# wcy199705/DfFintheWild

Hardware: AMD Instinct MI355X
Metric: focal-stacks/sec (10x3x256x256) (higher is better)
Workload: dtype bf16x3 (split-bf16 MFMA operands hi+lo, fp32 accumulate, fp32-accurate); 1 GPU; DFF_net forward, 10-slice 3x256x256 focal stacks, batch 32 per GPU (BASELINE.json config 3), dense focus_dists, synthetic weights seed 0; batch_per_gpu=32, global_batch=32, slices=10, height=256, width=256, parallelism=single GPU, precision=bf16x3, input=float32 (B,3,N,H,W), the reference's tensor contract

## Files before the change

dffinthewild_amd/csrc/dffw_conv_tile.h:

```cpp
#pragma once
#include "dffw_internal.h"

namespace dffw {

enum Geo {
    G3S1 = 0,
    G3S2 = 1,
    G3T = 2,
    G2S1 = 3,
    G2D = 4,
    G2S2 = 5,
    G2P = 6,
    GEO_COUNT = 6
};

struct GeoInfo {
    int minz, maxz, miny, maxy, minx, maxx;
    int s;
    int os;
    int npass;
};

inline GeoInfo geo_info(int geo) {
    switch (geo) {
        case G3S1: return GeoInfo{-1, 1, -1, 1, -1, 1, 1, 1, 1};
        case G3S2: return GeoInfo{-1, 1, -1, 1, -1, 1, 2, 1, 1};
        case G3T: return GeoInfo{-1, 1, 0, 1, 0, 1, 1, 2, 4};
        case G2D: return GeoInfo{0, 0, -8, 8, -6, 10, 1, 1, 1};
        case G2S2: return GeoInfo{0, 0, -1, 1, -1, 1, 2, 1, 1};
        case G2P: return GeoInfo{0, 0, -8, 8, -6, 10, 1, 1, 1};
        default: return GeoInfo{0, 0, -1, 1, -1, 1, 1, 1, 1};
    }
}

struct TileCfg {
    int id;
    int geo, nt, cg;
    int tz, ty, tx;
    int fz, fy, fx, fxl;
    int pipe;
    int nw;
    int kt;
    bool lean;
};

struct TileArgs {
    int npass, nstage;
    int KC[4];
    const int *tab[4];
    const uint16_t *wpk[4];
    int ooy[4], oox[4];
    int tiles_z, tiles_y, tiles_x;
    int total_tiles;
    int nt_total;
    int nsplit;
    int grid;
    int pass_split;
    int ksplit;
    float *partial;
    int64_t partial_stride;
    int warm;
};

enum class TileVariant { PLAIN, LEAN, SPLITK, RAW, SUMS };
constexpr int TILE_VARIANTS = 5;

const TileCfg *tile_cfg_find(int geo, int nt, int cg, bool wide = false);
const TileCfg *tile_cfg_find_shape(int geo, int nt, int cg, int tz, int ty, int tx);
const TileCfg *tile_cfg_find_like(const TileCfg *base, int nt);
const TileCfg *tile_cfg_find_team(const TileCfg *base, int nstage, int nt);
bool tile_cfg_has_splitk(const TileCfg *c);
bool tile_cfg_has_sums(const TileCfg *c);
int tile_cfg_count();
const TileCfg *tile_cfg_at(int i);
hipError_t launch_conv_tile(int prec, const TileCfg *cfg, const ConvArgs &a, const TileArgs &t, hipStream_t s);
void conv_tile_kernel_name(int prec, const TileCfg *cfg, const ConvArgs &a, const TileArgs &t, char *buf, int n);

}
```

dffinthewild_amd/csrc/dffw_conv_tile.hip:

```cpp
#include <cstdio>
#include <cstdlib>
#include <initializer_list>

#include "dffw_conv_geom.h"

#ifndef DFFW_TILE_PREC
#error "compile with -DDFFW_TILE_PREC=0|1|2 (arithmetic of this object, see the Makefile)"
#endif

namespace dffw {

template <int PREC, int GEO, int NT, int TZ, int TY, int TX, int CG, int PIPE, int NWAVES = 4, bool SPLITK = false, bool LEAN = false, int KT = 1>
__global__ __launch_bounds__(NWAVES * KT * 64) void conv_tile(const ConvArgs a, const TileArgs t) {
    using T = TileT<GEO, TZ, TY, TX, CG>;
    using G = GeoT<GEO>;
    constexpr int PARTS = Fmt<PREC>::PARTS;
    constexpr bool F16 = (PREC == P_FP16);
    constexpr int MTW = T::MT / NWAVES;
    constexpr bool STEM = (GEO == G2D || GEO == G2P);
    constexpr bool STEMP = (GEO == G2P);
    constexpr bool SUMS = (GEO == G2S1) && SPLITK;
    constexpr int CG8 = CG / 8;

    constexpr int PIXB = CG * 2;
    constexpr int PLANEB = (T::FPIX * PIXB + 1023) / 1024 * 1024;
    constexpr int LDSB = PARTS * PLANEB;
    static_assert(PLANEB < 65536, "lo-plane offset must fit the ds_read immediate");
    static_assert(KT == 1 || (!SPLITK && GEO != G2D && GEO != G2P), "teams: conv geometries (the transposed conv only with its passes split over grid.z), no split-K / raw variants");
    static_assert(KT * LDSB <= 160 * 1024, "the teams' LDS images must fit one CU");
    __shared__ __attribute__((aligned(1024))) unsigned char smem_all[KT * LDSB];

    const int team = KT > 1 ? (int)threadIdx.x / (NWAVES * 64) : 0;
    unsigned char *const smem = smem_all + team * LDSB;
    const int tid = KT > 1 ? (int)threadIdx.x % (NWAVES * 64) : (int)threadIdx.x;
    const int lane = tid & 63;
    const int wave = tid >> 6;
    const int g = lane >> 4, r = lane & 15;
    const int ntb = blockIdx.y * NT;
    const int NTT = t.nt_total;

    int tile;
    {
        const int bid = blockIdx.x;
        const int xcd = bid & 7, idx = bid >> 3;
        const int q = t.total_tiles >> 3, rem = t.total_tiles & 7;
        const int xs = xcd < rem ? xcd * (q + 1) : rem * (q + 1) + (xcd - rem) * q;
        const int xe = xs + q + (xcd < rem ? 1 : 0);
        tile = xs + idx;
        if (tile >= xe) return;
    }

    struct Coord {
        int b, gz0, gy0, gx0;
    };
    auto decode = [&](int tile) {
        Coord c;
        const int txi = tile % t.tiles_x;
        int tt = tile / t.tiles_x;
        const int tyi = tt % t.tiles_y;
        tt /= t.tiles_y;
        const int tzi = tt % t.tiles_z;
        c.b = tt / t.tiles_z;
        c.gz0 = tzi * TZ;
        c.gy0 = tyi * TY;
        c.gx0 = txi * TX;
        return c;
    };

    int pofs[MTW], voff[MTW], tcrd[MTW];
    const int lanepart = (PARTS == 2) ? (g & 1) * a.Cout + (g >> 1) * 8 : g * 4;
#pragma unroll
    for (int j = 0; j < MTW; ++j) {
        const int p = (wave * MTW + j) * 16 + r;
        if constexpr (STEMP) {
            constexpr int HP = TX / 2;
            const int k = p % HP, ty = (p / HP) % TY, tz = p / (HP * TY);
            const int tx = (k & 1) + 4 * (k >> 1) + 2 * (g >> 1);
            pofs[j] = ((tz * T::FY + ty) * T::FXL + k) * PIXB;
            voff[j] = ((tz * a.Ho + ty) * a.Wo + tx) * (PARTS * 8) + ((PARTS == 2) ? (g & 1) * 8 : (g & 1) * 4);
            tcrd[j] = tx | (ty << 8) | (tz << 16);
        } else {
            const int tx = p % TX, ty = (p / TX) % TY, tz = p / (TX * TY);
            pofs[j] = ((tz * T::FY + ty * G::S) * T::FXL + tx) * PIXB;
// ... 142 lines not shown
                uint32_t hh[4], ll[4];
                Fmt<PREC>::split2(px(0, iy, q - 2), px(1, iy, q - 2), hh[0], ll[0]);
                Fmt<PREC>::split2(px(2, iy, q - 2), 0.f, hh[1], ll[1]);
                Fmt<PREC>::split2(px(0, iy, q), px(1, iy, q), hh[2], ll[2]);
                Fmt<PREC>::split2(px(2, iy, q), 0.f, hh[3], ll[3]);
                h = __builtin_bit_cast(short8, (u32x4v){hh[0], hh[1], hh[2], hh[3]});
                l = __builtin_bit_cast(short8, (u32x4v){ll[0], ll[1], ll[2], ll[3]});
            }
            *reinterpret_cast<short8 *>(smem + p * PIXB) = h;
            if constexpr (PARTS == 2) *reinterpret_cast<short8 *>(smem + PLANEB + p * PIXB) = l;
        }
    };
    bool from_stack = false;
    if constexpr (STEM) from_stack = STEMP || a.fs32 != nullptr;
    if (from_stack) {
        if constexpr (STEM) fill_from_stack(cur);
    } else if (!(a.dbg & 1)) {
        issue_fill(cur, st_lo);
    }
    if (t.warm) {
        uint32_t sink = 0;
        const int wstride = NTT * PARTS * 64;
        for (int pass = pass_lo; pass < pass_hi; ++pass) {
            const int KCp = t.KC[pass];
            const int nlines = (st_hi - st_lo) * KCp * NT * PARTS * 8;
            const unsigned char *wb = reinterpret_cast<const unsigned char *>(t.wpk[pass]);
            if (tid * 128 < KCp * 16) {
                const unsigned char *p = reinterpret_cast<const unsigned char *>(t.tab[pass]) + tid * 128;
                asm volatile("global_load_dword %0, %1, off" : "+v"(sink) : "v"(p));
            }
            for (int i = tid; i < nlines; i += NWAVES * 64) {
                const int l8 = i & 7, f = (i >> 3) % (NT * PARTS), c = (i >> 3) / (NT * PARTS);
                const int kc = c % KCp, st = st_lo + c / KCp;
                const unsigned char *p = wb + ((((int64_t)st * KCp + kc) * wstride + ntb * PARTS * 64 + f * 64) * 16 + l8 * 128);
                asm volatile("global_load_dword %0, %1, off" : "+v"(sink) : "v"(p));
            }
        }
        asm volatile("s_waitcnt vmcnt(0)" : "+v"(sink)::"memory");
    }
    stamp(1);

    {
        f32x4 acc[NT][MTW];
#pragma unroll 1
        for (int pass = pass_lo; pass < pass_hi; ++pass) {
#pragma unroll
            for (int nt = 0; nt < NT; ++nt)
#pragma unroll
                for (int j = 0; j < MTW; ++j) acc[nt][j] = (BIAS_IN_ACC && !splitk && team == 0) ? bias4[nt] : f32x4{0.f, 0.f, 0.f, 0.f};

            const int KC = t.KC[pass];
            const int *tab = t.tab[pass] + g;

            for (int sti = st_lo; sti < st_hi; ++sti) {
                const bool backwards = (GEO == G3T) && ((pass - pass_lo) & 1);
                const int st = backwards ? st_hi - 1 - (sti - st_lo) : sti;
                const bool resident = (GEO == G3T) && pass > pass_lo && sti == st_lo && st_hi - st_lo > 1;
                const bool prefilled = (pass == pass_lo && sti == st_lo);
                const int wstride = NTT * PARTS * 64;
                const short8 *wp = reinterpret_cast<const short8 *>(t.wpk[pass]) + (int64_t)st * KC * wstride + ntb * PARTS * 64 + lane;
                short8 wfirst[NT][PARTS];
#pragma unroll
                for (int nt = 0; nt < NT; ++nt)
#pragma unroll
                    for (int pt = 0; pt < PARTS; ++pt) wfirst[nt][pt] = wp[(nt * PARTS + pt) * 64];
                const int tfirst = tab[0];
                constexpr int WD = KT > 1 ? 4 : 1;
                short8 wr[WD][NT][PARTS];
                int tr[WD];
                if constexpr (KT > 1) {
#pragma unroll
                    for (int q = 0; q < WD; ++q) {
                        const int kq = q < KC ? q : KC - 1;
#pragma unroll
                        for (int nt = 0; nt < NT; ++nt)
#pragma unroll
                            for (int pt = 0; pt < PARTS; ++pt) wr[q][nt][pt] = wp[(int64_t)kq * wstride + (nt * PARTS + pt) * 64];
                        tr[q] = tab[kq * 4];
                    }
                }
                if ((pass == pass_lo || st_hi - st_lo > 1) && !resident && !(a.dbg & 1)) {
                    if (!prefilled) {
                        __syncthreads();
                        issue_fill(cur, st);
                    }
                    asm volatile("s_waitcnt vmcnt(0)" ::: "memory");
                    __syncthreads();
                    if (prefilled) stamp(2);
                }

                if constexpr (PIPE == 0) {
                    short8 wf[NT][PARTS], wn[NT][PARTS];
                    int toff = tfirst, tn = 0;
    #pragma unroll
                    for (int nt = 0; nt < NT; ++nt)
    #pragma unroll
                        for (int pt = 0; pt < PARTS; ++pt) wf[nt][pt] = wfirst[nt][pt];
                    for (int kc = 0; kc < ((a.dbg & 2) ? 1 : KC); ++kc) {
                        if (kc + 1 < KC) {
    #pragma unroll
                            for (int nt = 0; nt < NT; ++nt)
    #pragma unroll
                                for (int pt = 0; pt < PARTS; ++pt) wn[nt][pt] = wp[(int64_t)(kc + 1) * wstride + (nt * PARTS + pt) * 64];
                            tn = tab[(kc + 1) * 4];
                        }
    #pragma unroll
// ... 433 lines not shown
    X(9, G3T, 1, 5, 4, 16, 16, 0, 4, 1)    \
    X(10, G3T, 2, 5, 4, 16, 16, 1, 4, 1)   \
    X(11, G3T, 4, 5, 4, 16, 16, 1, 4, 1)   \
    X(12, G2S1, 1, 5, 4, 16, 8, 0, 4, 1)   \
    X(13, G2S1, 1, 5, 4, 16, 16, 0, 4, 1)  \
    X(14, G2S1, 2, 5, 8, 16, 16, 1, 4, 1)  \
    X(15, G2D, 1, 1, 16, 32, 8, 0, 4, 1)   \
    X(16, G3S1, 2, 4, 4, 8, 16, 1, 4, 1)   \
    X(17, G3S2, 2, 4, 4, 8, 8, 1, 4, 1)    \
    X(18, G2S1, 2, 5, 4, 16, 8, 1, 4, 1)   \
    X(19, G2S1, 4, 5, 4, 16, 16, 1, 4, 1)  \
    X(20, G2S1, 4, 5, 4, 16, 8, 1, 4, 1)   \
    X(21, G2S2, 1, 5, 4, 16, 8, 0, 4, 1)   \
    X(22, G2S2, 2, 5, 4, 16, 8, 0, 4, 1)   \
    X(23, G3T, 1, 5, 4, 16, 32, 0, 4, 1)   \
    X(24, G3T, 2, 5, 4, 16, 32, 1, 4, 1)   \
    X(25, G3T, 4, 5, 4, 16, 32, 1, 4, 1)   \
    X(34, G2S1, 2, 5, 4, 16, 32, 1, 4, 1)  \
    X(37, G3S2, 4, 4, 4, 8, 16, 1, 4, 1)   \
    X(38, G3S2, 2, 4, 4, 8, 16, 1, 4, 1)   \
    X(39, G3S2, 1, 4, 4, 8, 16, 1, 4, 1)   \
    X(32, G2P, 1, 1, 16, 32, 8, 0, 4, 1)   \
    X(40, G3S1, 1, 5, 8, 8, 16, 1, 4, 1)   \
    X(41, G3S1, 2, 5, 8, 8, 16, 1, 4, 1)   \
    X(42, G3S1, 4, 5, 8, 8, 16, 1, 4, 1)   \
    X(43, G3T, 1, 5, 8, 8, 32, 0, 4, 1)    \
    X(44, G3T, 2, 5, 8, 8, 32, 1, 4, 1)    \
    X(45, G3T, 4, 5, 8, 8, 32, 1, 4, 1)
#define DFFW_TILE_CONFIGS_W8(X)            \
    X(26, G3S1, 1, 5, 8, 16, 16, 1, 8, 1)  \
    X(27, G3T, 1, 5, 8, 16, 16, 0, 8, 1)   \
    X(28, G2S1, 1, 5, 8, 16, 8, 0, 8, 1)   \
    X(29, G2S1, 1, 5, 8, 16, 16, 0, 8, 1)  \
    X(30, G2S1, 2, 5, 8, 16, 16, 0, 8, 1)  \
    X(31, G2D, 1, 1, 32, 32, 8, 0, 8, 1)   \
    X(33, G2P, 1, 1, 32, 32, 8, 0, 8, 1)

#define DFFW_TILE_CONFIGS_TEAM(X)           \
    X(50, G3S1, 1, 1, 4, 16, 16, 1, 2, 2)   \
    X(51, G3S1, 1, 1, 4, 16, 16, 1, 2, 4)   \
    X(52, G3S2, 1, 1, 4, 16, 8, 1, 2, 2)    \
    X(53, G3S2, 1, 1, 4, 16, 8, 1, 2, 4)    \
    X(58, G3T, 1, 1, 4, 16, 32, 1, 2, 2)    \
    X(59, G3T, 1, 1, 4, 16, 32, 1, 2, 4)    \
    X(60, G3T, 2, 1, 4, 16, 32, 1, 2, 2)    \
    X(61, G3T, 2, 1, 4, 16, 32, 1, 2, 4)
#define DFFW_TILE_CONFIGS_ALL(X) DFFW_TILE_CONFIGS(X) DFFW_TILE_CONFIGS_W8(X) DFFW_TILE_CONFIGS_TEAM(X)
constexpr int TILE_IDS = 64;

#define DFFW_TILE_IDS_SPLITK 0, 1, 2, 16, 5, 6, 17, 38, 39
#define DFFW_TILE_IDS_SUMS 34, 19
#define DFFW_TILE_IDS_RAW 15, 31, 32, 33
#define DFFW_TILE_IDS_NO_LEAN 23, 27

template <int ID>
struct TileTuple;
#define X_TUPLE(ID, GEO, NT, TZ, TY, TX, CG, PIPE, NW, KT) \
    template <>                                            \
    struct TileTuple<ID> { static constexpr int geo = GEO, nt = NT, tz = TZ, ty = TY, tx = TX, cg = CG, pipe = PIPE, nw = NW, kt = KT; };
DFFW_TILE_CONFIGS_ALL(X_TUPLE)
#undef X_TUPLE

struct TileRow {
    char name[80];
    void (*fn)(ConvArgs, TileArgs);
    int block;
    TileVariant variant;
};
struct TileIndex {
    const TileRow *at[3][TILE_VARIANTS][TILE_IDS];
};

template <int PREC, int ID, TileVariant V>
static const TileRow *tile_row() {
    using C = TileTuple<ID>;
    constexpr bool STEM = C::geo == G2D || C::geo == G2P;
    constexpr bool SPLITK = V == TileVariant::SPLITK || V == TileVariant::RAW || V == TileVariant::SUMS, LEAN = V == TileVariant::LEAN;
    static_assert(ID < TILE_IDS, "raise TILE_IDS");
    static_assert(V != TileVariant::LEAN || PREC == P_BF16X3, "LEAN exists in split-bf16 only");
    static_assert((V == TileVariant::SUMS) == (SPLITK && C::geo == G2S1) && (V == TileVariant::RAW) == (SPLITK && STEM), "what SPLITK = true means is the geometry's");
    static const TileRow row = [] {
        TileRow r;
        snprintf(r.name, sizeof r.name, "dffw::conv_tile<%d, %d, %d, %d, %d, %d, %d, %d, %d, %s, %s, %d>", PREC, C::geo, C::nt, C::tz, C::ty, C::tx, C::cg, C::pipe,
                 C::nw, SPLITK ? "true" : "false", LEAN ? "true" : "false", C::kt);
        r.fn = conv_tile<PREC, C::geo, C::nt, C::tz, C::ty, C::tx, C::cg, C::pipe, C::nw, SPLITK, LEAN, C::kt>;
        r.block = 64 * C::nw * C::kt;
        r.variant = V;
        return r;
    }();
    return &row;
}
template <int PREC, TileVariant V, int... IDS>
static void tile_rows(TileIndex &ix) {
    ((ix.at[PREC][(int)V][IDS] = tile_row<PREC, IDS, V>()), ...);
}

#define X_ID(ID, ...) , ID
#ifdef DFFW_TILE_LEAN
void tile_rows_lean0(TileIndex &ix) { tile_rows<P_BF16X3, TileVariant::LEAN DFFW_TILE_CONFIGS_ALL(X_ID)>(ix); }
#else
#define DFFW_CAT2(a, b) a##b
#define DFFW_CAT(a, b) DFFW_CAT2(a, b)
void DFFW_CAT(tile_rows_prec, DFFW_TILE_PREC)(TileIndex &ix) {
    tile_rows<DFFW_TILE_PREC, TileVariant::PLAIN DFFW_TILE_CONFIGS_ALL(X_ID)>(ix);
    tile_rows<DFFW_TILE_PREC, TileVariant::SPLITK, DFFW_TILE_IDS_SPLITK>(ix);
    tile_rows<DFFW_TILE_PREC, TileVariant::SUMS, DFFW_TILE_IDS_SUMS>(ix);
    tile_rows<DFFW_TILE_PREC, TileVariant::RAW, DFFW_TILE_IDS_RAW>(ix);
}
#endif
#undef X_ID

#if DFFW_TILE_PREC == 0 && !defined(DFFW_TILE_LEAN)
void tile_rows_prec1(TileIndex &ix);
void tile_rows_prec2(TileIndex &ix);
void tile_rows_lean0(TileIndex &ix);
static const TileIndex &tile_index() {
    static const TileIndex ix = [] {
        TileIndex ix = {};
        tile_rows_prec0(ix);
        tile_rows_prec1(ix);
        tile_rows_prec2(ix);
        tile_rows_lean0(ix);
        return ix;
    }();
    return ix;
}
static const TileRow *tile_row_of(int prec, TileVariant v, const TileCfg *c) {
    return c && (prec == P_BF16X3 || prec == P_FP16 || prec == P_BF16) ? tile_index().at[prec][(int)v][c->id] : nullptr;
}
bool tile_cfg_has_splitk(const TileCfg *c) { return tile_row_of(P_BF16X3, TileVariant::SPLITK, c) != nullptr; }
bool tile_cfg_has_sums(const TileCfg *c) { return tile_row_of(P_BF16X3, TileVariant::SUMS, c) != nullptr; }

constexpr bool tile_id_in(int id, std::initializer_list<int> ids) {
    for (int i : ids)
        if (i == id) return true;
    return false;
}
#define X_CFG(ID, GEO, NT, TZ, TY, TX, CG, PIPE, NW, KT)                                                     \
    TileCfg{ID, GEO, NT, CG, TZ, TY, TX, TileT<GEO, TZ, TY, TX, CG>::FZ, TileT<GEO, TZ, TY, TX, CG>::FY, \
            TileT<GEO, TZ, TY, TX, CG>::FX, TileT<GEO, TZ, TY, TX, CG>::FXL, PIPE, NW, KT, !tile_id_in(ID, {DFFW_TILE_IDS_NO_LEAN})},
static const TileCfg g_cfgs[] = {DFFW_TILE_CONFIGS_ALL(X_CFG)};
#undef X_CFG

int tile_cfg_count() { return (int)(sizeof(g_cfgs) / sizeof(g_cfgs[0])); }
const TileCfg *tile_cfg_at(int i) { return (i >= 0 && i < tile_cfg_count()) ? &g_cfgs[i] : nullptr; }
const TileCfg *tile_cfg_find(int geo, int nt, int cg, bool wide) {
    if (wide)
        for (const TileCfg &c : g_cfgs)
            if (c.nw == 8 && c.kt <= 1 && c.geo == geo && c.nt == nt && c.cg == cg) return &c;
    for (const TileCfg &c : g_cfgs)
        if (c.nw == 4 && c.kt <= 1 && c.geo == geo && c.nt == nt && c.cg == cg) return &c;
    return nullptr;
}

const TileCfg *tile_cfg_find_shape(int geo, int nt, int cg, int tz, int ty, int tx) {
    for (const TileCfg &c : g_cfgs)
        if (c.nw == 4 && c.kt <= 1 && c.geo == geo && c.nt == nt && c.cg == cg && c.tz == tz && c.ty == ty && c.tx == tx) return &c;
    return nullptr;
}

const TileCfg *tile_cfg_find_like(const TileCfg *base, int nt) {
    for (const TileCfg &c : g_cfgs)
        if (c.kt <= 1 && c.geo == base->geo && c.cg == base->cg && c.nt == nt && c.tz == base->tz && c.ty == base->ty && c.tx == base->tx && c.nw == base->nw) return &c;
    return nullptr;
}

const TileCfg *tile_cfg_find_team(const TileCfg *base, int nstage, int nt) {
    for (const TileCfg &c : g_cfgs)
        if (c.kt == nstage && c.kt > 1 && c.geo == base->geo && c.cg == base->cg && c.nt == nt && c.ty == base->ty && c.tx == base->tx) return &c;
    return nullptr;
}

static const TileRow *select_tile(int prec, const TileCfg *c, const ConvArgs &a, const TileArgs &t) {
    if (!c) return nullptr;
    const bool lean = prec == P_BF16X3 && t.ksplit <= 1 && !(a.dbg & (DFFW_ARGS_RAW | DFFW_ARGS_SUMS)) && (a.out || a.out_pre || a.cls_w) && !a.outf && !a.res1 &&
                      !a.res_bcast && a.relu != 2 && (a.Cout == t.nt_total * 16 || (a.Cout == 8 && c->nt == 1)) && !(a.dbg & DFFW_ARGS_NO_LEAN_TILE) && c->lean;
    const TileVariant v = lean                        ? TileVariant::LEAN
                          : t.ksplit > 1              ? TileVariant::SPLITK
                          : (a.dbg & DFFW_ARGS_SUMS) ? TileVariant::SUMS
                          : (a.dbg & DFFW_ARGS_RAW)  ? TileVariant::RAW
                                                      : TileVariant::PLAIN;
    return tile_row_of(prec, v, c);
}

static dim3 tile_grid(TileVariant v, const TileArgs &t) {
    switch (v) {
        case TileVariant::SPLITK: return dim3((unsigned)t.grid, (unsigned)t.nsplit, (unsigned)t.ksplit);
        case TileVariant::SUMS: return dim3((unsigned)t.grid, 1, 1);
        case TileVariant::RAW: return dim3((unsigned)t.grid, (unsigned)t.nsplit, 1);
        default: return dim3((unsigned)t.grid, (unsigned)t.nsplit, (unsigned)(t.pass_split ? 4 : 1));
    }
}

hipError_t launch_conv_tile(int prec, const TileCfg *cfg, const ConvArgs &a, const TileArgs &t, hipStream_t s) {
    const TileRow *row = select_tile(prec, cfg, a, t);
    if (!row) return hipErrorInvalidValue;
    if (cfg->kt > 1 && (t.nstage != cfg->kt || t.ksplit > 1 || (cfg->geo == G3T && !t.pass_split))) return hipErrorInvalidValue;
    hipLaunchKernelGGL(row->fn, tile_grid(row->variant, t), dim3(row->block), 0, s, a, t);
    return hipGetLastError();
}

void conv_tile_kernel_name(int prec, const TileCfg *cfg, const ConvArgs &a, const TileArgs &t, char *buf, int n) {
    const TileRow *row = select_tile(prec, cfg, a, t);
    if (n > 0) snprintf(buf, n, "%s", row ? row->name : "");
}
#endif

}
```

dffinthewild_amd/csrc/dffw_dispatch.cpp:

```cpp
#include "dffw_run.h"
#include "dffw_stem.h"

namespace dffw {
namespace {

struct ConvLaunch {
    char kernel[96];
    const char *suffix;
    ConvArgs a;
    RollArgs r;
    int v0, v1;
    double flops, bytes;
};

enum { F_TILE = 100, F_GATHER = 101 };

struct ConvPlan {
    int family = -1;
    int n = 0;
    ConvLaunch l[4];
    bool clear_scores = false;
    const TileCfg *cfg = nullptr;
    TileArgs t;
    bool stem_pipe = false;
// ... 265 lines not shown
        t.grid = 8 * ((t.total_tiles + 7) / 8);
        t.warm = (t.total_tiles * t.nsplit <= sw.warm_max_wgs) ? 1 : 0;
    };
    auto team_wgs = [&](const TileCfg *c, int nsplit, int npass) {
        return (int64_t)a.B * ((a.Ng + c->tz - 1) / c->tz) * ((a.Hg + c->ty - 1) / c->ty) * ((a.Wg + c->tx - 1) / c->tx) * nsplit * npass;
    };
    set_tiles(cfg);
    const int split_below = (cfg->geo == G3T && pc.nt >= 4) ? sw.split_t64 : (cfg->geo == G3S1 && pc.nt == 4) || (cfg->geo == G3S2 && pc.nt >= 8) ? sw.split_s64 : ((cfg->geo == G3S1 || cfg->geo == G3T) ? 257 : 256);
    if (t.total_tiles < split_below && pc.nt > 1 && !o.cls && !sw.on(SW_NO_SPLIT)) {
        const int want = (256 + t.total_tiles - 1) / t.total_tiles;
        for (int nts = pc.nt / 2; nts >= 1; nts /= 2) {
            const TileCfg *c2 = pc.nt % nts == 0 ? tile_cfg_find_like(tp.cfg, nts) : nullptr;
            if (!c2) continue;
            cfg = c2;
            t.nsplit = pc.nt / nts;
            if (t.nsplit >= want) break;
        }
        set_tiles(cfg);
    }
    t.ksplit = 1;
    p.M_out = (int64_t)out.B * No * Ho * Wo;
    const int thr = sw.split_wg;
    t.pass_split = (L.transposed && t.total_tiles * t.nsplit <= thr && !sw.on(SW_NO_SPLITK)) ? 1 : 0;
    if (t.pass_split && tp.nstage >= 2 && !sw.on(SW_NO_TEAMS)) {
        for (int nts = cfg->nt; nts <= pc.nt && nts <= 2; nts *= 2) {
            const TileCfg *team = pc.nt % nts == 0 ? tile_cfg_find_team(cfg, tp.nstage, nts) : nullptr;
            if (!team || team_wgs(team, pc.nt / nts, 4) > sw.team_max_wgs) continue;
            cfg = team;
            t.nsplit = pc.nt / nts;
            set_tiles(cfg);
            break;
        }
    }
    if (!t.pass_split && tile_cfg_has_splitk(cfg) && t.total_tiles * t.nsplit <= thr * 3 / 4 && tp.nstage >= 2 && !o.cls && !o.out_pre && !o.outf && !o.discard && !o.res_bcast && L.cout % 4 == 0 &&
        !sw.on(SW_NO_SPLITK)) {
        const int want = (sw.ksplit_target + t.total_tiles * t.nsplit - 1) / (t.total_tiles * t.nsplit);
        t.ksplit = std::max(1, std::min(std::min(tp.nstage, want), 8));
        const TileCfg *team = (t.ksplit > 1 && !sw.on(SW_NO_TEAMS)) ? tile_cfg_find_team(cfg, tp.nstage, cfg->nt) : nullptr;
        if (team) {
            const int64_t wgs = team_wgs(team, t.nsplit, 1);
            if (wgs < sw.team_min_wgs || wgs > sw.team_max_wgs) team = nullptr;
        }
        if (team) {
            cfg = team;
            t.ksplit = 1;
            set_tiles(cfg);
        }
        if (t.ksplit > 1) {
            t.partial_stride = p.M_out * (int64_t)pc.nt * 16;
            p.partial_bytes = t.ksplit * t.partial_stride * (int64_t)sizeof(float);
            p.finish_bytes = (double)p.M_out * L.cout * (4.0 * t.ksplit + eb * (o.res0 ? 2 : 1));
        }
    }
    p.stem_pipe = stem_pair && !sw.on(SW_NO_STEM_PIPE) && !sw.tracing(name) && stem_pipe_ok(prec, cfg, a, t);
    p.family = F_TILE;
    p.cfg = cfg;
    p.n = 1;
    ConvLaunch &l = p.l[0];
    l.a = a;
    l.suffix = "";
    l.flops = flops;
    l.bytes = in_b + (o.outf ? opx * L.cout * 4.0 : out_b(o.out_pre ? 2 : 1)) + out_b(res(o.res0) + res(o.res1)) + w_b((double)L.kd * L.kh * L.kw);
    if (p.stem_pipe) stem_pipe_kernel_name(a, l.kernel, sizeof l.kernel);
    else conv_tile_kernel_name(prec, cfg, a, t, l.kernel, sizeof l.kernel);
}

void Planner::gather(ConvPlan &p) {
    p.family = F_GATHER;
    for (const Variant &v : pc.variants) {
        a.KC = v.KC;
        a.tab = v.tab;
        a.wpk = v.wpk;
        if (L.transposed) {
            a.Ng = in0.N; a.Hg = in0.H; a.Wg = in0.W;
            a.sy = a.sx = 1;
            a.osy = a.osx = 2;
            a.ooy = v.ooy; a.oox = v.oox;
        } else {
            a.Ng = No; a.Hg = Ho; a.Wg = Wo;
            a.sy = L.sh; a.sx = L.sw;
            a.osy = a.osx = 1;
            a.ooy = a.oox = 0;
        }
        a.M = (int64_t)a.B * a.Ng * a.Hg * a.Wg;
        if (sw.on(SW_NO_SMALL)) a.dbg |= DFFW_ARGS_NO_SMALL;
        ConvLaunch &l = p.l[p.n++];
        l.a = a;
        l.suffix = "";
        conv_kernel_name_for(prec, a, l.kernel, 64);
        const double nv = (double)pc.variants.size();
        const double px = (double)a.M;
        l.flops = 2.0 * (double)a.M * v.ntaps * L.cin * L.cout;
        l.bytes = in_b / nv
                  + px * L.cout * (o.outf ? 4.0 : eb * (o.out_pre ? 2 : 1))
                  + px * L.cout * eb * (res(o.res0) + res(o.res1))
                  + (double)v.ntaps * L.cin * L.cout * eb;
    }
}

void plan_conv(const std::string &name, const PackedConv &pc, const PackedConv *cls, const Act &in0, const ConvOpt &o, const Act &out, const Switches &sw,
               int prec, ConvPlan &p) {
    const LayerDef &L = pc.def;
    const int No = out.N, Ho = out.H, Wo = out.W;
    auto reject = [&](const char *fmt, const char *x, const char *y) {
        p.err = DFFW_EINVAL;
        snprintf(p.msg, sizeof p.msg, fmt, x, y);
// ... 142 lines not shown
```

dffinthewild_amd/csrc/dffw_run.h:

```cpp
#pragma once
#include <algorithm>
#include <climits>
#include <cstdio>
#include <cstdlib>
#include <cstring>
#include <initializer_list>
#include <map>
#include <string>
#include <vector>

#include "../../include/dffw.h"
#include "dffw_align.h"
#include "dffw_conv_roll.h"
#include "dffw_conv_tile.h"
#include "dffw_internal.h"
#include "dffw_pack.h"

void dffw_set_last_conv_kernel(const char *name);

extern "C" char **environ;

namespace dffw {

static constexpr auto &fail = dffw_fail;
// ... 65 lines not shown

struct dffw_engine {
    int device = 0, net = 0, prec = 0;
    std::map<std::string, dffw::PackedConv> convs;
    dffw::RepackPlan *repack = nullptr;
    bool profiling = false;
    std::vector<ProfRec> recs;
    uint16_t *zero_page = nullptr;
    static constexpr int NSIDE = 2, NEV = 16;
    hipStream_t side[NSIDE] = {nullptr, nullptr};
    hipEvent_t ev[NEV] = {};
    int ensure_side() {
        if (side[0]) return DFFW_OK;
        for (int i = 0; i < NSIDE; ++i) HIPCHK(hipStreamCreateWithFlags(&side[i], hipStreamNonBlocking));
        for (int i = 0; i < NEV; ++i) HIPCHK(hipEventCreateWithFlags(&ev[i], hipEventDisableTiming));
        return DFFW_OK;
    }
    int ensure_zero_page() {
        if (zero_page) return DFFW_OK;
        HIPCHK(hipMalloc((void **)&zero_page, 256));
        HIPCHK(hipMemset(zero_page, 0, 256));
        return DFFW_OK;
    }
    void clear_recs() {
        for (auto &r : recs) {
            if (r.e0) (void)hipEventDestroy(r.e0);
            if (r.e1) (void)hipEventDestroy(r.e1);
        }
        recs.clear();
    }
    ~dffw_engine() {
        clear_recs();
        if (zero_page) (void)hipFree(zero_page);
        for (int i = 0; i < NSIDE; ++i)
            if (side[i]) (void)hipStreamDestroy(side[i]);
        for (int i = 0; i < NEV; ++i)
            if (ev[i]) (void)hipEventDestroy(ev[i]);
        for (auto &kv : convs) dffw::free_packed(kv.second);
        dffw::free_repack_plan(repack);
    }
};

namespace dffw {

inline bool getenv_flag(const char *name) {
    const char *v = getenv(name);
    return v && *v && *v != '0';
}

#define DFFW_SWITCHES(X)                                                                                                 \
    X(NO_CONCURRENT) X(NO_CONF_FORK) X(NO_FUSED_ATTENTION) X(NO_FUSED_EFD) X(NO_FUSED_OF) X(NO_FUSED_POOL) X(NO_FUSED_SRD) \
    X(NO_FUSED_STEM) X(NO_HEAD_SPLIT) X(NO_ROLL) X(NO_ROLL_S2) X(NO_SPLIT) X(NO_SPLITK)  \
    X(NO_STEM_PAIR) X(NO_TILE) X(NO_SMALL) X(NO_ROLL_S2_WIDE) X(NO_HEAD_SUMS) X(NO_HEAD_SUMS_FUSED) X(NO_HEAD_WARP) X(NO_OF_FIRST) \
    X(NO_LEAN_TILE) X(NO_LEAN_ROLL) X(NO_ROLLX) X(NO_ROLLK) X(NO_ROLLT) X(NO_TEAMS) X(NO_SLICE32) X(NO_REGRESS_FUSED) X(NO_STEM_PIPE) X(NO_POOL3) X(NO_NARROW)
enum SwitchId {
#define X_ID(n) SW_##n,
    DFFW_SWITCHES(X_ID)
#undef X_ID
    SW_COUNT
};
#define DFFW_INT_KNOBS(X)                                                                                                                                  \
    X(ROLL_WGS, roll_wgs, 8, 0)                                                                                                                            \
    X(SRD_WGS, srd_wgs, 8, 0)                                                                                                                              \
                                                                                                                                         \
    X(SMALL_MAX_UNITS, small_max_units, 0, 0)                                                                                                              \
    X(ROLL_ZSPLIT, roll_zsplit, 1, 0)                                                                                                                      \
    X(KSPLIT_TARGET, ksplit_target, 1, 512)                                                                                                                \
                                                                  \
    X(REDIR_SIDE, redir_side, 0, -1)                                                                                                                       \
    X(TEAM_MIN_WGS, team_min_wgs, 0, 0)                                                                                                                    \
    X(TEAM_MAX_WGS, team_max_wgs, 1, 320)                                                                                                                  \
     \
    X(SPLIT_S64, split_s64, 1, 1025)                                                                                                                       \
                                                 \
    X(SPLIT_T64, split_t64, 1, 1025)                                                                                                                       \
                                   \
    X(NARROW_MAX, narrow_max, 1, 40)                                                                                                                       \
                                      \
    X(WARM_MAX_WGS, warm_max_wgs, 0, 1024)                                                                                                                 \
                                                                                            \
    X(ROLLK_MERGE_BELOW, rollk_merge_below, 0, 1 << 30)                                                                                                    \
                                                                                                \
    X(ROLLT_MIN_UNITS, rollt_min_units, 1, 128)                                                                                                            \
                                                                                                                \
    X(ROLL_MIN_UNITS, roll_min_units, 1, 192)                                                                                                              \
                                                                                                     \
    X(SPLIT_WG, split_wg, INT_MIN, 256)                                                                                                                    \
                        \
    X(WGRAD_WGS, wgrad_wgs, 8, 0)                                                                                                                          \
    X(WGRAD_FLUSH_UNITS, wgrad_flush_units, 1, 256)                                                                                                        \
                                                                 \
    X(PWGRAD_WGS, pwgrad_wgs, 8, 0)                                                                                                                        \
    X(PWGRAD_FLUSH_STEPS, pwgrad_flush_steps, 1, 512)                                                                                                      \
                                                                                                                       \
    X(BN_WGS, bn_wgs, 1, 0)                                                                                                                                \
                                                                                               \
    X(SCORE_WGS, score_wgs, 1, 0)                                                                                                                          \
    X(DEBUG_FLAGS, debug_flags, INT_MIN, 0)
#define DFFW_INT64_KNOBS(X)                                                                                                                                \
                                                                                                                                        \
    X(CONCURRENT_MAX_PIXELS, concurrent_max_pixels, -1)                                                                                                    \
                            \
    X(CONCURRENT_MIN_PIXELS, concurrent_min_pixels, 400000)

inline void warn_unknown_switches() {
    static const bool once = [] {
        static const char *const known[] = {
#define X_NM(n) "DFFW_" #n,
            DFFW_SWITCHES(X_NM)
#undef X_NM
#define X_NM(n, ...) "DFFW_" #n,
            DFFW_INT_KNOBS(X_NM) DFFW_INT64_KNOBS(X_NM)
#undef X_NM
            "DFFW_SRD_PIPE", "DFFW_TRACE_LAYER", "DFFW_TRACE_OUT", "DFFW_RCCL_LIB", "DFFW_LIB_PATH", "DFFW_NO_PROBE", "DFFW_PRECISION",
            "DFFW_BENCH_ONE_DEVICE", "DFFW_BENCH_TIMEOUT_S",
            "DFFW_SRD_ABL", "DFFW_ROLLX_ABL", "DFFW_ROLLX_NTS", "DFFW_ROLLK_ABL", "DFFW_ROLLK_SKEW"};
        for (char **e = ::environ; e && *e; ++e) {
            if (strncmp(*e, "DFFW_", 5) != 0) continue;
            const char *eq = strchr(*e, '=');
            const size_t n = eq ? (size_t)(eq - *e) : strlen(*e);
            bool ok = false;
            for (const char *k : known) ok = ok || (strlen(k) == n && strncmp(k, *e, n) == 0);
            if (!ok) fprintf(stderr, "libdffw: environment variable %.*s is not a switch this library reads (retired or misspelt?) -- ignored\n", (int)n, *e);
        }
        return true;
    }();
    (void)once;
}

struct Switches {
    bool f[SW_COUNT];
#define X_FIELD(n, field, lo, dflt) int field = dflt;
    DFFW_INT_KNOBS(X_FIELD)
#undef X_FIELD
// ... 323 lines not shown
```

Baseline: 4159 stacks/s.

## Add double-buffered LDS overlap variant for small-grid 3x3x3 split-bf16 conv tiles

Adds a PIPE==2 variant of the conv tile kernel for 3x3x3 split-bf16 single-team configurations. It keeps two LDS input images, so the next channel stage is filled with global_load_lds while the current stage's MFMAs run. Weights stream through a 7-deep register ring with explicit vmcnt/lgkmcnt waits. Dispatch picks this variant only when the tile grid is at most 256 workgroups, the case where per-stage fill latency is exposed. In exchange it doubles the LDS footprint, which can cut occupancy, and adds register pressure from the ring and the double-buffered operands.

```diff
diff --git a/dffinthewild_amd/csrc/dffw_conv_tile.h b/dffinthewild_amd/csrc/dffw_conv_tile.h
--- a/dffinthewild_amd/csrc/dffw_conv_tile.h
+++ b/dffinthewild_amd/csrc/dffw_conv_tile.h
@@ -60,6 +60,7 @@
     float *partial;
     int64_t partial_stride;
     int warm;
+    int overlap;
 };
 
 enum class TileVariant { PLAIN, LEAN, SPLITK, RAW, SUMS };
@@ -71,6 +72,7 @@
 const TileCfg *tile_cfg_find_team(const TileCfg *base, int nstage, int nt);
 bool tile_cfg_has_splitk(const TileCfg *c);
 bool tile_cfg_has_sums(const TileCfg *c);
+bool tile_overlap_ok(int prec, const TileCfg *c, const ConvArgs &a, const TileArgs &t);
 int tile_cfg_count();
 const TileCfg *tile_cfg_at(int i);
 hipError_t launch_conv_tile(int prec, const TileCfg *cfg, const ConvArgs &a, const TileArgs &t, hipStream_t s);
diff --git a/dffinthewild_amd/csrc/dffw_conv_tile.hip b/dffinthewild_amd/csrc/dffw_conv_tile.hip
--- a/dffinthewild_amd/csrc/dffw_conv_tile.hip
+++ b/dffinthewild_amd/csrc/dffw_conv_tile.hip
@@ -28,7 +28,10 @@
     static_assert(PLANEB < 65536, "lo-plane offset must fit the ds_read immediate");
     static_assert(KT == 1 || (!SPLITK && GEO != G2D && GEO != G2P), "teams: conv geometries (the transposed conv only with its passes split over grid.z), no split-K / raw variants");
     static_assert(KT * LDSB <= 160 * 1024, "the teams' LDS images must fit one CU");
-    __shared__ __attribute__((aligned(1024))) unsigned char smem_all[KT * LDSB];
+    constexpr bool OVL = (PIPE == 2);
+    static_assert(!OVL || ((GEO == G3S1 || GEO == G3S2) && KT == 1 && !SPLITK && PARTS == 2 && 2 * LDSB + NWAVES * 1024 <= 160 * 1024), "overlap: 3x3x3 split-bf16 configurations, one team, two images in one CU's LDS");
+    constexpr int NIMG = OVL ? 2 : KT;
+    __shared__ __attribute__((aligned(1024))) unsigned char smem_all[NIMG * LDSB + (OVL ? NWAVES * 1024 : 0)];
 
     const int team = KT > 1 ? (int)threadIdx.x / (NWAVES * 64) : 0;
     unsigned char *const smem = smem_all + team * LDSB;
@@ -277,6 +280,151 @@
             const int KC = t.KC[pass];
             const int *tab = t.tab[pass] + g;
 
+            if constexpr (OVL) {
+                constexpr int KCC = (27 * CG8 + 3) / 4;
+                constexpr int WD = 7;
+                static_assert(KCC % WD == 0, "ring slots must not shift from stage to stage");
+                constexpr int PPW = 64 / CG8, STEP = PPW * NWAVES, NPI = (T::FPIX + STEP - 1) / STEP;
+                constexpr int FPC = (NPI + KCC - 1) / KCC, NGF = (NPI + FPC - 1) / FPC;
+                constexpr int CNT = FPC * PARTS + NT * PARTS + 1;
+                constexpr int WAITW = (WD - 2) * CNT < 63 ? (WD - 2) * CNT : 63;
+                constexpr int WAITI = (KCC - NGF) * CNT < 63 ? (KCC - NGF) * CNT : 63;
+                const unsigned lds0 = (unsigned)(uintptr_t)(__attribute__((address_space(3))) unsigned char *)smem;
+                const int nst = st_hi - st_lo, total = nst * KCC;
+                const unsigned wsb = (unsigned)(NTT * PARTS * 64) * 16u;
+                const unsigned wofs0 = ((unsigned)st_lo * KCC) * wsb + (unsigned)(ntb * PARTS * 64 + lane) * 16u;
+                const unsigned char *const wbase = reinterpret_cast<const unsigned char *>(t.wpk[0]);
+                const int *const tbase = t.tab[0];
+                short8 wr[WD][NT][PARTS];
+                int tr[WD];
+                short8 x[2][MTW][PARTS];
+                unsigned pofl[MTW];
+#pragma unroll
+                for (int j = 0; j < MTW; ++j) pofl[j] = lds0 + (unsigned)pofs[j];
+
+                auto ring_load_ = [](auto Q, short8 (&wr)[WD][NT][PARTS], int (&tr)[WD], int f, int kc, int total, unsigned wofs0, unsigned wsb, const unsigned char *wbase, const int *tbase, int g) __attribute__((always_inline)) {
+                    constexpr int q = decltype(Q)::value;
+                    const bool in = f < total;
+                    const unsigned fo = wofs0 + (unsigned)(in ? f : total - 1) * wsb;
+#pragma unroll
+                    for (int nt = 0; nt < NT; ++nt)
+#pragma unroll
+                        for (int pt = 0; pt < PARTS; ++pt) {
+                            const unsigned o = fo + (unsigned)((nt * PARTS + pt) * 1024);
+                            asm volatile("global_load_dwordx4 %0, %1, %2" : "=v"(wr[q][nt][pt]) : "v"(o), "s"(wbase) : "memory");
+                        }
+                    const unsigned to = (unsigned)(((in ? kc : KCC - 1) * 4 + g) * 4);
+                    asm volatile("global_load_dword %0, %1, %2" : "=v"(tr[q]) : "v"(to), "s"(tbase) : "memory");
+                };
+                auto ring_tie_ = [](auto Q, short8 (&wr)[WD][NT][PARTS], int (&tr)[WD]) __attribute__((always_inline)) {
+                    constexpr int q = decltype(Q)::value;
+#pragma unroll
+                    for (int nt = 0; nt < NT; ++nt)
+#pragma unroll
+                        for (int pt = 0; pt < PARTS; ++pt) asm volatile("" : "+v"(wr[q][nt][pt]));
+                    asm volatile("" : "+v"(tr[q]));
+                };
+                const int iz0 = cur.gz0 + G::MINZ, iy0 = cur.gy0 * G::S + G::MINY, ix0 = cur.gx0 * G::S + G::MINX;
+                const bool yx_in = iy0 >= 0 && iy0 + T::FY <= a.Hi && ix0 >= 0 && ix0 + T::FX <= a.Wi;
+                auto fill_piece = [&](int st, int it, int imgb, bool live) __attribute__((always_inline)) {
+                    const int pbase = (it * NWAVES + wave) * PPW;
+                    const bool real = live && it < NPI && pbase < T::FPIX;
+                    const uint16_t *gp = a.zero;
+                    int pstep = 0;
+                    if (real) {
+                        const int ch = st * CG + (lane % CG8) * 8;
+                        const bool second = ch >= a.C0;
+                        const int cc = second ? ch - a.C0 : ch;
+                        const int csrc = second ? a.C1 : a.C0;
+                        const uint16_t *sp = second ? a.in1 + cur.b * samp1 : a.in0 + cur.b * samp0;
+                        const int p = pbase + lane / CG8;
+                        const int lx = p % T::FXL, fy = (p / T::FXL) % T::FY, fz = p / (T::FXL * T::FY);
+                        const int fx = (G::S == 2) ? (lx < T::FXL / 2 ? 2 * lx : 2 * (lx - T::FXL / 2) + 1) : lx;
+                        const int iz = iz0 + fz, iy = iy0 + fy, ix = ix0 + fx;
+                        bool ok = ((unsigned)iz < (unsigned)a.Ni) & (p < T::FPIX);
+                        if (T::FXL > T::FX) ok = ok & (fx < T::FX);
+                        if (!yx_in) ok = ok & ((unsigned)iy < (unsigned)a.Hi) & ((unsigned)ix < (unsigned)a.Wi);
+                        if (ok) {
+                            gp = sp + ((int64_t)(((iz * a.Hi + iy) * a.Wi + ix) * (PARTS * csrc)) + cc);
+                            pstep = csrc;
+                        }
+                    }
+                    const int dst = real ? imgb + pbase * PIXB : 2 * LDSB + wave * 1024;
+#pragma unroll
+                    for (int part = 0; part < PARTS; ++part) {
+                        const uint16_t *src = gp + part * pstep;
+                        asm volatile("" : "+v"(src));
+                        __builtin_amdgcn_global_load_lds((const __attribute__((address_space(1))) void *)src,
+                                                         (__attribute__((address_space(3))) void *)(smem + dst + (real ? part * PLANEB : 0)), 16, 0, 0);
+                    }
+                };
+                auto fetch_ = [](auto B, short8 (&x)[2][MTW][PARTS], const unsigned (&pofl)[MTW], unsigned toff) __attribute__((always_inline)) {
+                    constexpr int b = decltype(B)::value;
+#pragma unroll
+                    for (int j = 0; j < MTW; ++j) {
+                        const unsigned ad = pofl[j] + toff;
+                        asm volatile("ds_read_b128 %0, %1" : "=v"(x[b][j][0]) : "v"(ad));
+                        asm volatile("ds_read_b128 %0, %1 offset:%2" : "=v"(x[b][j][1]) : "v"(ad), "n"(PLANEB));
+                    }
+                };
+                auto x_tie_ = [](auto B, short8 (&x)[2][MTW][PARTS]) __attribute__((always_inline)) {
+                    constexpr int b = decltype(B)::value;
+#pragma unroll
+                    for (int j = 0; j < MTW; ++j) asm volatile("" : "+v"(x[b][j][0]), "+v"(x[b][j][1]));
+                };
+
+                auto ring_load = [&](auto Q, int f, int kc) __attribute__((always_inline)) { ring_load_(Q, wr, tr, f, kc, total, wofs0, wsb, wbase, tbase, g); };
+                auto ring_tie = [&](auto Q) __attribute__((always_inline)) { ring_tie_(Q, wr, tr); };
+                auto fetch = [&](auto B, unsigned toff) __attribute__((always_inline)) { fetch_(B, x, pofl, toff); };
+                auto x_tie = [&](auto B) __attribute__((always_inline)) { x_tie_(B, x); };
+                static_for<WD>([&](auto Q) __attribute__((always_inline)) { ring_load(Q, decltype(Q)::value, decltype(Q)::value % KCC); });
+                asm volatile("s_waitcnt vmcnt(0)" ::: "memory");
+                __builtin_amdgcn_sched_barrier(0);
+                static_for<WD>([&](auto Q) __attribute__((always_inline)) { ring_tie(Q); });
+
+                for (int si = 0; si < nst; ++si) {
+                    const int st = st_lo + si;
+                    const int imgc = (si & 1) * LDSB, imgn = LDSB - imgc;
+                    const bool has_next = si + 1 < nst;
+                    const int f0 = si * KCC;
+                    asm volatile("s_waitcnt vmcnt(%0)" ::"n"(WAITI) : "memory");
+                    asm volatile("s_waitcnt lgkmcnt(0)\n\ts_barrier" ::: "memory");
+                    if (si == 0) stamp(2);
+                    fetch(std::integral_constant<int, 0>{}, (unsigned)(tr[0] + imgc));
+                    static_for<KCC>([&](auto C) __attribute__((always_inline)) {
+                        constexpr int c = decltype(C)::value;
+                        constexpr int q = c % WD, q1 = (c + 1) % WD, cb = c & 1;
+                        asm volatile("s_waitcnt vmcnt(%0)" ::"n"(WAITW) : "memory");
+                        __builtin_amdgcn_sched_barrier(0);
+                        ring_tie(std::integral_constant<int, q1>{});
+                        asm volatile("s_waitcnt lgkmcnt(0)" ::: "memory");
+                        __builtin_amdgcn_sched_barrier(0);
+                        x_tie(std::integral_constant<int, cb>{});
+                        if constexpr (c + 1 < KCC) fetch(std::integral_constant<int, cb ^ 1>{}, (unsigned)(tr[q1] + imgc));
+                        __builtin_amdgcn_sched_barrier(0);
+#pragma unroll
+                        for (int j = 0; j < MTW; ++j)
+#pragma unroll
+                            for (int nt = 0; nt < NT; ++nt) acc[nt][j] = mma<F16>(wr[q][nt][1], x[cb][j][0], acc[nt][j]);
+#pragma unroll
+                        for (int j = 0; j < MTW; ++j)
+#pragma unroll
+                            for (int nt = 0; nt < NT; ++nt) acc[nt][j] = mma<F16>(wr[q][nt][0], x[cb][j][1], acc[nt][j]);
+#pragma unroll
+                        for (int j = 0; j < MTW; ++j)
+#pragma unroll
+                            for (int nt = 0; nt < NT; ++nt) acc[nt][j] = mma<F16>(wr[q][nt][0], x[cb][j][0], acc[nt][j]);
+                        __builtin_amdgcn_sched_barrier(0);
+#pragma unroll
+                        for (int i = 0; i < FPC; ++i) fill_piece(st + 1, c * FPC + i, imgn, has_next);
+                        ring_load(std::integral_constant<int, q>{}, f0 + c + WD, (c + WD) % KCC);
+                        __builtin_amdgcn_sched_barrier(0);
+                    });
+                }
+                asm volatile("s_waitcnt vmcnt(0)" ::: "memory");
+                __builtin_amdgcn_sched_barrier(0);
+                static_for<WD>([&](auto Q) __attribute__((always_inline)) { ring_tie(Q); });
+            } else
             for (int sti = st_lo; sti < st_hi; ++sti) {
                 const bool backwards = (GEO == G3T) && ((pass - pass_lo) & 1);
                 const int st = backwards ? st_hi - 1 - (sti - st_lo) : sti;
@@ -816,6 +964,7 @@
 #define DFFW_TILE_IDS_SUMS 34, 19
 #define DFFW_TILE_IDS_RAW 15, 31, 32, 33
 #define DFFW_TILE_IDS_NO_LEAN 23, 27
+#define DFFW_TILE_IDS_OVERLAP 0, 2, 5, 6, 16, 17, 38, 39, 41
 
 template <int ID>
 struct TileTuple;
@@ -833,6 +982,7 @@
 };
 struct TileIndex {
     const TileRow *at[3][TILE_VARIANTS][TILE_IDS];
+    const TileRow *overlap[TILE_IDS];
 };
 
 template <int PREC, int ID, TileVariant V>
@@ -858,10 +1008,28 @@
 static void tile_rows(TileIndex &ix) {
     ((ix.at[PREC][(int)V][IDS] = tile_row<PREC, IDS, V>()), ...);
 }
+template <int ID>
+static const TileRow *tile_row_overlap() {
+    using C = TileTuple<ID>;
+    static_assert(C::pipe == 1 && C::kt == 1, "overlap: a variant of the software-pipelined single-team configurations");
+    static const TileRow row = [] {
+        TileRow r = *tile_row<P_BF16X3, ID, TileVariant::LEAN>();
+        r.fn = conv_tile<P_BF16X3, C::geo, C::nt, C::tz, C::ty, C::tx, C::cg, 2, C::nw, false, true, 1>;
+        return r;
+    }();
+    return &row;
+}
+template <int... IDS>
+static void tile_rows_overlap(TileIndex &ix) {
+    ((ix.overlap[IDS] = tile_row_overlap<IDS>()), ...);
+}
 
 #define X_ID(ID, ...) , ID
 #ifdef DFFW_TILE_LEAN
-void tile_rows_lean0(TileIndex &ix) { tile_rows<P_BF16X3, TileVariant::LEAN DFFW_TILE_CONFIGS_ALL(X_ID)>(ix); }
+void tile_rows_lean0(TileIndex &ix) {
+    tile_rows<P_BF16X3, TileVariant::LEAN DFFW_TILE_CONFIGS_ALL(X_ID)>(ix);
+    tile_rows_overlap<DFFW_TILE_IDS_OVERLAP>(ix);
+}
 #else
 #define DFFW_CAT2(a, b) a##b
 #define DFFW_CAT(a, b) DFFW_CAT2(a, b)
@@ -944,7 +1112,18 @@
                           : (a.dbg & DFFW_ARGS_SUMS) ? TileVariant::SUMS
                           : (a.dbg & DFFW_ARGS_RAW)  ? TileVariant::RAW
                                                       : TileVariant::PLAIN;
+    if (t.overlap && v == TileVariant::LEAN && tile_index().overlap[c->id]) return tile_index().overlap[c->id];
     return tile_row_of(prec, v, c);
+}
+
+bool tile_overlap_ok(int prec, const TileCfg *c, const ConvArgs &a, const TileArgs &t) {
+    if (!c || c->kt > 1 || !tile_index().overlap[c->id] || t.nstage < 2 || t.ksplit > 1 || t.pass_split || t.npass != 1 || (a.dbg & 3)) return false;
+    const int planeb = (c->fz * c->fy * c->fxl * c->cg * 2 + 1023) / 1024 * 1024;
+    if (2 * 2 * planeb + c->nw * 1024 > 160 * 1024 || t.KC[0] != (27 * (c->cg / 8) + 3) / 4) return false;
+    TileArgs one = t;
+    one.overlap = 0;
+    const TileRow *row = select_tile(prec, c, a, one);
+    return row && row->variant == TileVariant::LEAN;
 }
 
 static dim3 tile_grid(TileVariant v, const TileArgs &t) {
diff --git a/dffinthewild_amd/csrc/dffw_dispatch.cpp b/dffinthewild_amd/csrc/dffw_dispatch.cpp
--- a/dffinthewild_amd/csrc/dffw_dispatch.cpp
+++ b/dffinthewild_amd/csrc/dffw_dispatch.cpp
@@ -341,6 +341,7 @@
             p.finish_bytes = (double)p.M_out * L.cout * (4.0 * t.ksplit + eb * (o.res0 ? 2 : 1));
         }
     }
+    t.overlap = (!sw.on(SW_NO_TILE_OVERLAP) && (int64_t)t.total_tiles * t.nsplit <= sw.tile_overlap_max_wgs && tile_overlap_ok(prec, cfg, a, t)) ? 1 : 0;
     p.stem_pipe = stem_pair && !sw.on(SW_NO_STEM_PIPE) && !sw.tracing(name) && stem_pipe_ok(prec, cfg, a, t);
     p.family = F_TILE;
     p.cfg = cfg;
diff --git a/dffinthewild_amd/csrc/dffw_run.h b/dffinthewild_amd/csrc/dffw_run.h
--- a/dffinthewild_amd/csrc/dffw_run.h
+++ b/dffinthewild_amd/csrc/dffw_run.h
@@ -141,7 +141,8 @@
     X(NO_CONCURRENT) X(NO_CONF_FORK) X(NO_FUSED_ATTENTION) X(NO_FUSED_EFD) X(NO_FUSED_OF) X(NO_FUSED_POOL) X(NO_FUSED_SRD) \
     X(NO_FUSED_STEM) X(NO_HEAD_SPLIT) X(NO_ROLL) X(NO_ROLL_S2) X(NO_SPLIT) X(NO_SPLITK)  \
     X(NO_STEM_PAIR) X(NO_TILE) X(NO_SMALL) X(NO_ROLL_S2_WIDE) X(NO_HEAD_SUMS) X(NO_HEAD_SUMS_FUSED) X(NO_HEAD_WARP) X(NO_OF_FIRST) \
-    X(NO_LEAN_TILE) X(NO_LEAN_ROLL) X(NO_ROLLX) X(NO_ROLLK) X(NO_ROLLT) X(NO_TEAMS) X(NO_SLICE32) X(NO_REGRESS_FUSED) X(NO_STEM_PIPE) X(NO_POOL3) X(NO_NARROW)
+    X(NO_LEAN_TILE) X(NO_LEAN_ROLL) X(NO_ROLLX) X(NO_ROLLK) X(NO_ROLLT) X(NO_TEAMS) X(NO_SLICE32) X(NO_REGRESS_FUSED) X(NO_STEM_PIPE) X(NO_POOL3) X(NO_NARROW) \
+    X(NO_TILE_OVERLAP)
 enum SwitchId {
 #define X_ID(n) SW_##n,
     DFFW_SWITCHES(X_ID)
@@ -169,6 +170,8 @@
     X(WARM_MAX_WGS, warm_max_wgs, 0, 1024)                                                                                                                 \
                                                                                             \
     X(ROLLK_MERGE_BELOW, rollk_merge_below, 0, 1 << 30)                                                                                                    \
+                                                                                                                                    \
+    X(TILE_OVERLAP_MAX_WGS, tile_overlap_max_wgs, 0, 256)                                                                                                    \
                                                                                                 \
     X(ROLLT_MIN_UNITS, rollt_min_units, 1, 128)                                                                                                            \
                                                                                                                 \
```

New measurement: 4185 stacks/s (median of 6 runs). About the same (+0.6%).
